# JiaruiFeng/KP-GNN

Measured on AMD Instinct MI355X. Metric: graphs/sec KP-GIN fwd+bwd, ZINC-12k K=8 L=8 h=104, higher is better.
Workload: dtype f32; 1 GPU; ZINC-12k-shaped synthetic molecules, KPGINPlus K=8 L=8 h=104 kernel=spd geometric combine, fwd+bwd+Adam, L1 loss; global_batch=2048, nodes_per_batch=47450, khop_edges_per_batch=1018372, active_pairs_per_batch=1018372, parallelism=dp1, launch=hipGraph replay of fwd+bwd, batches=4 pre-staged batches cycled

## Files before the change

include/kpgnn.h:

```cpp
#ifndef KPGNN_H_
#define KPGNN_H_

#include <stddef.h>
#include <stdint.h>

#ifdef __cplusplus
extern "C" {
#endif

#define KPGNN_ABI_VERSION 1

#define KPGNN_OK 0
#define KPGNN_EINVAL (-1)
#define KPGNN_EHIP (-2)
#define KPGNN_ELIMIT (-3)

typedef void* kpgnn_stream_t;

int kpgnn_abi_version(void);
const char* kpgnn_last_error(void);

int kpgnn_device_info(int* cu_count, int* lds_bytes_per_block, int* wavefront, char* arch, int arch_len);


// ... 341 lines not shown

#define KPGNN_STAT_REPLICAS 8
size_t kpgnn_stat_slot_bytes(int32_t C);

typedef struct kpgnn_wgrad_desc {
    int64_t N;
    int32_t O, I;
    const float* dy; int64_t dy_stride;
    const float* x;  int64_t x_stride;
    float* dw;
    float* db;
    void* workspace; size_t workspace_bytes;
    const float* x_mean; const float* x_invstd; const float* x_gamma; const float* x_beta;
    int32_t x_relu;
    kpgnn_reduce_job* defer;
    const float* dy_mask;
    const int32_t* n_dyn;
    int32_t math;
} kpgnn_wgrad_desc;

size_t kpgnn_wgrad_workspace_bytes(int32_t O, int32_t I);
int kpgnn_linear_wgrad(const kpgnn_wgrad_desc* d, kpgnn_stream_t stream);
int kpgnn_linear_wgrad_pair(const kpgnn_wgrad_desc* a, const kpgnn_wgrad_desc* b, kpgnn_stream_t stream);
size_t kpgnn_wgrad_group_workspace_bytes(int32_t O, int32_t I, int32_t group);
int kpgnn_linear_wgrad_group(const kpgnn_wgrad_desc* d, const float* const* x_group, int32_t group, kpgnn_stream_t stream);

typedef struct kpgnn_linear_desc {
    int64_t N;
    int32_t O, I;
    const float* x; int64_t x_stride;
    const float* w;
    const float* bias;
    float* y; int64_t y_stride;
    int32_t w_transposed;
    int32_t y_block_cols; int64_t y_block_stride;
    const float* x_mask;
    const int32_t* n_dyn;
    int32_t math;
    void* workspace; size_t workspace_bytes;
} kpgnn_linear_desc;

int kpgnn_linear_fwd(const kpgnn_linear_desc* d, kpgnn_stream_t stream);
size_t kpgnn_linear_split_workspace_bytes(int32_t O, int32_t I, int32_t group);
typedef struct kpgnn_split_job { const float* w; int64_t wn, wk; int32_t O, I; void* frag; } kpgnn_split_job;
int kpgnn_linear_split_many(const kpgnn_split_job* jobs, int32_t n, kpgnn_stream_t stream);

// ... 531 lines not shown
```

kp_gnn_amd/_lib.py:

```python
import ctypes
import os

import torch

_PKG = os.path.dirname(os.path.abspath(__file__))
HIP_LIB_PATH = os.path.join(_PKG, "libkpgnn_hip.so")

MODE_GIN, MODE_GINPLUS, MODE_GCN, MODE_SUM = 0, 1, 2, 3
ROUTE_SUBGROUP, ROUTE_NARROW, ROUTE_SMALL, ROUTE_LDS = 0, 1, 2, 3

c_i32, c_i64, c_f32p, c_vp = ctypes.c_int32, ctypes.c_int64, ctypes.c_void_p, ctypes.c_void_p


MATH_AUTO, MATH_F32 = 0, 1
ELIMIT = -3
DENSE_MATH = MATH_AUTO


class KpgnnError(RuntimeError):
    pass


class AggFwdDesc(ctypes.Structure):
    _fields_ = [
# ... 509 lines not shown
    "kpgnn_dict_grad_multi": (ctypes.c_int, [ctypes.POINTER(DictGradMultiDesc), c_vp]),
    "kpgnn_dict_grad_slabs": (c_i32, [c_i32]),
    "kpgnn_tile_pack_filter": (ctypes.c_int, [c_vp, c_vp, c_i64, c_i32, c_vp, c_vp, c_vp, c_vp]),
    "kpgnn_tile_pack_prefixes": (ctypes.c_int, [c_vp, c_vp, c_i64, c_i32, c_i64, c_vp, c_vp, c_vp, c_vp, c_i32, c_vp]),
    "kpgnn_collate": (ctypes.c_int, [ctypes.POINTER(CollateDesc), c_vp]),
    "kpgnn_regression_loss": (ctypes.c_int, [c_vp, c_vp, c_i64, c_i32, c_vp, c_vp, c_vp]),
    "kpgnn_score_head_fwd": (ctypes.c_int, [c_vp, c_vp, c_vp, c_i64, c_i32, c_vp, c_vp]),
    "kpgnn_score_head_bwd": (ctypes.c_int, [c_vp, c_vp, c_vp, c_i64, c_i32, c_vp, c_vp, c_vp, c_vp]),
    "kpgnn_adam_step": (ctypes.c_int, [c_vp, c_vp, c_vp, c_vp, c_i64, c_i64, ctypes.c_double, ctypes.c_double, ctypes.c_double,
                                       ctypes.c_double, ctypes.c_double, c_vp]),
    "kpgnn_reduce_jobs": (ctypes.c_int, [c_vp, c_i32, c_vp]),
    "kpgnn_adam_step_device": (ctypes.c_int, [c_vp, c_vp, c_vp, c_vp, c_i64, c_vp, ctypes.c_double, ctypes.c_double,
                                              ctypes.c_double, ctypes.c_double, ctypes.c_double, c_vp]),
    "kpgnn_multi_copy": (ctypes.c_int, [c_i32, c_vp, c_vp, c_vp, c_vp]),
    "kpgnn_dict_tile_pack": (ctypes.c_int, [c_vp, c_i64, c_i32, c_i32, c_i32, c_vp, c_vp]),
    "kpgnn_dict_tile_pack_dyn": (ctypes.c_int, [c_vp, c_i64, c_i32, c_vp, c_i32, c_i32, c_vp, c_vp]),
    "kpgnn_combine_bwd_workspace_bytes": (ctypes.c_size_t, [c_i32] * 3),
    "kpgnn_combine_bwd": (ctypes.c_int, [ctypes.POINTER(CombineBwdDesc), c_vp]),
    "kpgnn_bn_fwd": (ctypes.c_int, [ctypes.POINTER(BnDesc), c_vp]),
    "kpgnn_bn_bwd": (ctypes.c_int, [ctypes.POINTER(BnBwdDesc), c_vp]),
    "kpgnn_wgrad_workspace_bytes": (ctypes.c_size_t, [c_i32, c_i32]),
    "kpgnn_linear_wgrad": (ctypes.c_int, [ctypes.POINTER(WgradDesc), c_vp]),
    "kpgnn_linear_wgrad_pair": (ctypes.c_int, [ctypes.POINTER(WgradDesc), ctypes.POINTER(WgradDesc), c_vp]),
    "kpgnn_wgrad_group_workspace_bytes": (ctypes.c_size_t, [c_i32, c_i32, c_i32]),
    "kpgnn_linear_wgrad_group": (ctypes.c_int, [ctypes.POINTER(WgradDesc), c_vp, c_i32, c_vp]),
    "kpgnn_linear_bn": (ctypes.c_int, [ctypes.POINTER(LinearBnDesc), c_vp]),
    "kpgnn_mlp_eval": (ctypes.c_int, [ctypes.POINTER(MlpEvalDesc), c_vp]),
    "kpgnn_bn_eval": (ctypes.c_int, [ctypes.POINTER(BnEvalDesc), c_vp]),
    "kpgnn_enc_tables_fwd": (ctypes.c_int, [ctypes.POINTER(EncTablesDesc), c_vp]),
    "kpgnn_enc_tables_bwd": (ctypes.c_int, [ctypes.POINTER(EncTablesDesc), c_vp]),
    "kpgnn_segment_pool_fwd": (ctypes.c_int, [ctypes.POINTER(PoolDesc), c_vp]),
    "kpgnn_segment_pool_bwd": (ctypes.c_int, [ctypes.POINTER(PoolDesc), c_vp]),
    "kpgnn_segment_max_fwd": (ctypes.c_int, [ctypes.POINTER(PoolMaxDesc), c_vp]),
    "kpgnn_segment_max_bwd": (ctypes.c_int, [ctypes.POINTER(PoolMaxDesc), c_vp]),
    "kpgnn_resistance_distance": (ctypes.c_int, [ctypes.POINTER(RdDesc), c_vp]),
    "kpgnn_rd_large_workspace_bytes": (ctypes.c_size_t, [c_i32, c_i32]),
    "kpgnn_resistance_distance_large": (ctypes.c_int, [ctypes.POINTER(RdLargeDesc), c_vp]),
    "kpgnn_rd_proj_workspace_bytes": (ctypes.c_size_t, [c_i64, c_i32]),
    "kpgnn_rd_proj_fwd": (ctypes.c_int, [ctypes.POINTER(RdProjDesc), c_vp]),
    "kpgnn_rd_proj_bwd": (ctypes.c_int, [ctypes.POINTER(RdProjDesc), c_vp]),
    "kpgnn_khop_dev_workspace_bytes": (ctypes.c_size_t, [c_i64]),
    "kpgnn_khop_dev_count": (ctypes.c_int, [ctypes.POINTER(KhopDevDesc), c_vp]),
    "kpgnn_khop_dev_fill": (ctypes.c_int, [ctypes.POINTER(KhopDevDesc), c_vp]),
    "kpgnn_khop_large_workspace_bytes": (ctypes.c_size_t, [c_i64, c_i64, c_i32]),
    "kpgnn_khop_large_count": (ctypes.c_int, [ctypes.POINTER(KhopDevDesc), c_vp]),
    "kpgnn_khop_large_fill": (ctypes.c_int, [ctypes.POINTER(KhopDevDesc), c_vp]),
# ... 135 lines not shown
```

kp_gnn_amd/csrc/wgrad.hip:

```cpp
#include <cstdlib>
#include <type_traits>

#include "bf3.h"
#include "kpgnn_common.h"

namespace kpgnn {
namespace {

constexpr int kWgradBlocks = 512;

struct WgParams {
    int64_t N; int O, I;
    const float* dy; int64_t dys;
    const float* x; int64_t xs;
    const float* xm; const float* xi; const float* xg; const float* xb; int xrelu;
    float* slab;
    int64_t slab_row, slab_off;
};
struct WgPair { WgParams q[2]; };

template <int TI, int RG>
__device__ __forceinline__ void wgrad_problem(const WgParams p, float* lds) {
    const int lane = threadIdx.x & 63;
    const int nstrip = (int)(blockDim.x >> 6) / RG;
// ... 164 lines not shown
    switch (ti) {
        case 1: KP_WG(1); break;
        case 2: KP_WG(2); break;
        case 3: KP_WG(3); break;
        case 4: KP_WG(4); break;
        case 5: KP_WG(5); break;
        case 6: KP_WG(6); break;
        case 7: KP_WG(7); break;
        default: KP_WG(8); break;
    }
#undef KP_WG
    KPGNN_LAUNCH_CHECK("wgrad_kernel");
    return KPGNN_OK;
}

constexpr int kW2Rows = 32;
constexpr int kW2MaxProb = 16;

struct Wg2Prob {
    const float* dy; const float* x; const float* mask;
    const float* xm; const float* xi; const float* xg; const float* xb;
    int xrelu;
    int64_t dys, xs, out_off, bias_off;
};
struct Wg2Args {
    int64_t N; const int32_t* n_dyn;
    int O, I, nprob; int64_t ldw;
    float* slab; int64_t slab_row;
    Wg2Prob q[kW2MaxProb];
};

template <int TI>
__global__ void __launch_bounds__(256, 2)
wgrad2_kernel(const Wg2Args A) {
    extern __shared__ __attribute__((aligned(16))) float w2[];
    constexpr int R = kW2Rows;
    const int O = A.O, I = A.I;
    float* dyl = w2;
    float* xl = w2 + R * O;
    float* coef = xl + R * I;
    const int tid = threadIdx.x, wave = tid >> 6, lane = tid & 63;
    const int kk = lane >> 5, c = lane & 31;
    const int nprob = A.nprob;
    const int pi = (int)(blockIdx.x % nprob), slice = (int)(blockIdx.x / nprob), nslices = (int)(gridDim.x / nprob);
    Wg2Prob q = A.q[0];
#pragma unroll
    for (int i = 1; i < kW2MaxProb; ++i)
        if (pi == i) q = A.q[i];
    const int64_t N = A.n_dyn ? (int64_t)min((int64_t)*A.n_dyn, A.N) : A.N;
    const bool tr = q.xm != nullptr;
    if (tr)
// ... 57 lines not shown
#pragma unroll
    for (int t = 0; t < TI; ++t) bp[t] = xl + kk * I + min(t * 32 + c, I - 1);
    const int64_t chunks = (N + R - 1) / R;
    int64_t ch = slice;
    if (tr) __syncthreads();
    if (ch < chunks) { issue(ch); commit(ch); }
    __syncthreads();
    for (; ch < chunks; ch += nslices) {
        const int64_t nx = ch + nslices;
        const bool more = nx < chunks;
        if (more) issue(nx);
#pragma unroll
        for (int p2 = 0; p2 < R / 2; ++p2) {
            const float a = ap[2 * p2 * O];
            bsum += a;
#pragma unroll
            for (int t = 0; t < TI; ++t) acc[t] = __builtin_amdgcn_mfma_f32_32x32x2f32(a, bp[t][2 * p2 * I], acc[t], 0, 0, 0);
        }
        __syncthreads();
        if (more) commit(nx);
        __syncthreads();
    }
    bsum += __shfl_xor(bsum, 32);
    float* out = A.slab + (int64_t)slice * A.slab_row;
#pragma unroll
    for (int t = 0; t < TI; ++t) {
        const int i = t * 32 + c;
        for (int v = 0; v < 16; ++v) {
            const int orow = wave * 32 + (v & 3) + 8 * (v >> 2) + 4 * kk;
            if (orow < O && i < I) out[q.out_off + (int64_t)orow * A.ldw + i] = acc[t][v];
        }
    }
    if (q.bias_off >= 0 && kk == 0 && o_ok) out[q.bias_off + o] = bsum;
}

constexpr int kW3Pitch = 40;

constexpr int kW3Blocks = 256;

template <int TI, bool MASK>
__global__ void __launch_bounds__(512, 1)
wgrad3_kernel(const Wg2Args A) {
    extern __shared__ __attribute__((aligned(16))) float w2[];
    constexpr int R = kW2Rows, P = kW3Pitch;
    const int O = A.O, I = A.I;
    const int bufsz = 3 * (O + I) * P;
    __bf16* pl = reinterpret_cast<__bf16*>(w2);
    float* coef = reinterpret_cast<float*>(pl + 2 * bufsz);
    const int tid = threadIdx.x, lane = tid & 63;
    const int wave = __builtin_amdgcn_readfirstlane(tid >> 6);
    const int kg = lane >> 5, c = lane & 31;
    const int nprob = A.nprob;
    const int pi = (int)(blockIdx.x % nprob), slice = (int)(blockIdx.x / nprob), nslices = (int)(gridDim.x / nprob);
    Wg2Prob q = A.q[0];
#pragma unroll
    for (int i = 1; i < kW2MaxProb; ++i)
        if (pi == i) q = A.q[i];
    const int64_t N = A.n_dyn ? (int64_t)min((int64_t)*A.n_dyn, A.N) : A.N;
    const bool tr = q.xm != nullptr;
    if (tr)
        for (int i = tid; i < I; i += 512) { coef[i] = q.xm[i]; coef[I + i] = q.xi[i]; coef[2 * I + i] = q.xg[i]; coef[3 * I + i] = q.xb[i]; }
    const int64_t chunks = (N + R - 1) / R;
    const int64_t mine = slice < chunks ? (chunks - slice + nslices - 1) / nslices : 0;
    const bool producer = wave >= 4;
    const bool is_x = wave >= 6;
    const int ncg = (is_x ? I : O) >> 2;
    const int task = tid & 127;
    const bool owner = producer && task < 4 * ncg;
    const int g = owner ? task & 3 : 0, cg = owner ? task >> 2 : 0;
    const float* src = is_x ? q.x : q.dy;
    const int64_t sstride = is_x ? q.xs : q.dys;
    const uint32_t sbytes = (uint32_t)sstride * 4u;
    const bool xform = tr && is_x;
    const int64_t last = N - 1;
    bf3_f2 bs01 = {0.f, 0.f}, bs23 = {0.f, 0.f};
    auto produce = [&](auto mask_c) {
        constexpr bool M = decltype(mask_c)::value;
        float4 pv0[8], pm0[8], pv1[8], pm1[8];
        auto issue = [&](int64_t k, float4 (&pv)[8], float4 (&pm)[8]) {
            const int64_t c0 = (slice + min(k, mine - 1) * nslices) * R;
            const float* cp = src + c0 * sstride;
            const float* mp = M ? q.mask + c0 * sstride : nullptr;
            const int lim = (int)min((int64_t)R, N - c0) - 1;
#pragma unroll
            for (int j = 0; j < 8; ++j) {
                const uint32_t off = __umul24((uint32_t)min(8 * g + j, lim), sbytes) + 16u * (uint32_t)cg;
                pv[j] = *reinterpret_cast<const float4*>(reinterpret_cast<const char*>(cp) + off);
                if (M) pm[j] = *reinterpret_cast<const float4*>(reinterpret_cast<const char*>(mp) + off);
            }
        };
        auto commit = [&](int64_t k, float4 (&pv)[8], float4 (&pm)[8]) {
            const int64_t c0 = (slice + min(k, mine - 1) * nslices) * R;
            if (M) {
    #pragma unroll
                for (int j = 0; j < 8; ++j) {
                    pv[j].x = pm[j].x > 0.f ? pv[j].x : 0.f; pv[j].y = pm[j].y > 0.f ? pv[j].y : 0.f;
                    pv[j].z = pm[j].z > 0.f ? pv[j].z : 0.f; pv[j].w = pm[j].w > 0.f ? pv[j].w : 0.f;
                }
            }
            if (xform) {
                const float4 m4 = *reinterpret_cast<const float4*>(coef + 4 * cg), s4 = *reinterpret_cast<const float4*>(coef + I + 4 * cg);
                const float4 g4 = *reinterpret_cast<const float4*>(coef + 2 * I + 4 * cg), b4 = *reinterpret_cast<const float4*>(coef + 3 * I + 4 * cg);
    #pragma unroll
                for (int j = 0; j < 8; ++j) {
                    float4 v = pv[j];
                    v.x = fmaf((v.x - m4.x) * s4.x, g4.x, b4.x); v.y = fmaf((v.y - m4.y) * s4.y, g4.y, b4.y);
                    v.z = fmaf((v.z - m4.z) * s4.z, g4.z, b4.z); v.w = fmaf((v.w - m4.w) * s4.w, g4.w, b4.w);
                    if (q.xrelu) { v.x = fmaxf(v.x, 0.f); v.y = fmaxf(v.y, 0.f); v.z = fmaxf(v.z, 0.f); v.w = fmaxf(v.w, 0.f); }
                    pv[j] = v;
                }
            }
            if (c0 + R > N) {
    #pragma unroll
                for (int j = 0; j < 8; ++j)
                    if (c0 + 8 * g + j >= N) pv[j] = make_float4(0.f, 0.f, 0.f, 0.f);
            }
            if (!is_x && k < mine) {
    #pragma unroll
                for (int j = 0; j < 8; ++j) { bs01 += bf3_f2{pv[j].x, pv[j].y}; bs23 += bf3_f2{pv[j].z, pv[j].w}; }
            }
            if (owner) {
                __bf16* base = pl + (k & 1) * bufsz + (is_x ? 3 * O * P : 0) + 8 * g;
                const int cols = is_x ? I : O;
    #pragma unroll
                for (int e2 = 0; e2 < 2; ++e2) {
                    bf3_u2 h[8], m[8], l[8];
#pragma unroll
                    for (int j = 0; j < 8; ++j)
                        bf3_split2(e2 == 0 ? bf3_f2{pv[j].x, pv[j].y} : bf3_f2{pv[j].z, pv[j].w}, h[j], m[j], l[j]);
                    __bf16* col = base + (4 * cg + 2 * e2) * P;
                    *reinterpret_cast<uint4*>(col) = make_uint4(bf3_pack(h[0].x, h[1].x), bf3_pack(h[2].x, h[3].x), bf3_pack(h[4].x, h[5].x), bf3_pack(h[6].x, h[7].x));
                    *reinterpret_cast<uint4*>(col + P) = make_uint4(bf3_pack(h[0].y, h[1].y), bf3_pack(h[2].y, h[3].y), bf3_pack(h[4].y, h[5].y), bf3_pack(h[6].y, h[7].y));
                    *reinterpret_cast<uint4*>(col + cols * P) = make_uint4(bf3_pack(m[0].x, m[1].x), bf3_pack(m[2].x, m[3].x), bf3_pack(m[4].x, m[5].x), bf3_pack(m[6].x, m[7].x));
                    *reinterpret_cast<uint4*>(col + cols * P + P) = make_uint4(bf3_pack(m[0].y, m[1].y), bf3_pack(m[2].y, m[3].y), bf3_pack(m[4].y, m[5].y), bf3_pack(m[6].y, m[7].y));
                    *reinterpret_cast<uint4*>(col + 2 * cols * P) = make_uint4(bf3_pack(l[0].x, l[1].x), bf3_pack(l[2].x, l[3].x), bf3_pack(l[4].x, l[5].x), bf3_pack(l[6].x, l[7].x));
                    *reinterpret_cast<uint4*>(col + 2 * cols * P + P) = make_uint4(bf3_pack(l[0].y, l[1].y), bf3_pack(l[2].y, l[3].y), bf3_pack(l[4].y, l[5].y), bf3_pack(l[6].y, l[7].y));
                }
            }
        };
        __builtin_amdgcn_s_setprio(2);
        if (mine > 0) {
            issue(0, pv0, pm0);
            issue(1, pv1, pm1);
            commit(0, pv0, pm0);
            issue(2, pv0, pm0);
        }
        __syncthreads();
        for (int64_t k = 0; k < mine; k += 2) {
            commit(k + 1, pv1, pm1);
            issue(k + 3, pv1, pm1);
            __syncthreads();
            commit(k + 2, pv0, pm0);
            issue(k + 4, pv0, pm0);
            __syncthreads();
        }
    };
    f32x16 acc[TI];
#pragma unroll
    for (int t = 0; t < TI; ++t)
        for (int v = 0; v < 16; ++v) acc[t][v] = 0.f;
    const int o = wave * 32 + c;
    const bool strip = !producer && wave * 32 < O;
    const int aoff = min(o, O - 1) * P + 8 * kg;
    int boff[TI];
#pragma unroll
    for (int t = 0; t < TI; ++t) boff[t] = 3 * O * P + min(t * 32 + c, I - 1) * P + 8 * kg;
    auto ld8 = [&](const __bf16* ptr) { return __builtin_bit_cast(bf3_x8, *reinterpret_cast<const uint4*>(ptr)); };
    auto multiply = [&](int64_t k) {
        const __bf16* bf = pl + (k & 1) * bufsz;
#pragma unroll
        for (int ks = 0; ks < R / 16; ++ks) {
            const bf3_x8 ah = ld8(bf + aoff + 16 * ks), am = ld8(bf + aoff + O * P + 16 * ks), al = ld8(bf + aoff + 2 * O * P + 16 * ks);
            bf3_x8 bh[TI], bm[TI], bl[TI];
#pragma unroll
            for (int t = 0; t < TI; ++t) {
                bh[t] = ld8(bf + boff[t] + 16 * ks); bm[t] = ld8(bf + boff[t] + I * P + 16 * ks); bl[t] = ld8(bf + boff[t] + 2 * I * P + 16 * ks);
            }
#pragma unroll
            for (int t = 0; t < TI; ++t) acc[t] = __builtin_amdgcn_mfma_f32_32x32x16_bf16(al, bh[t], acc[t], 0, 0, 0);
#pragma unroll
            for (int t = 0; t < TI; ++t) acc[t] = __builtin_amdgcn_mfma_f32_32x32x16_bf16(ah, bl[t], acc[t], 0, 0, 0);
#pragma unroll
            for (int t = 0; t < TI; ++t) acc[t] = __builtin_amdgcn_mfma_f32_32x32x16_bf16(am, bm[t], acc[t], 0, 0, 0);
#pragma unroll
            for (int t = 0; t < TI; ++t) acc[t] = __builtin_amdgcn_mfma_f32_32x32x16_bf16(am, bh[t], acc[t], 0, 0, 0);
#pragma unroll
            for (int t = 0; t < TI; ++t) acc[t] = __builtin_amdgcn_mfma_f32_32x32x16_bf16(ah, bm[t], acc[t], 0, 0, 0);
#pragma unroll
            for (int t = 0; t < TI; ++t) acc[t] = __builtin_amdgcn_mfma_f32_32x32x16_bf16(ah, bh[t], acc[t], 0, 0, 0);
        }
    };
    if (tr) __syncthreads();
    float* out = A.slab + (int64_t)slice * A.slab_row;
    if (producer) {
        if (MASK && !is_x) produce(std::true_type{});
        else produce(std::false_type{});
    } else {
        __syncthreads();
        for (int64_t k = 0; k < mine; k += 2) {
            if (strip) multiply(k);

            __syncthreads();

            if (strip && k + 1 < mine) multiply(k + 1);

            __syncthreads();
        }
        if (strip) {
#pragma unroll
            for (int t = 0; t < TI; ++t) {
                const int i = t * 32 + c;
                for (int v = 0; v < 16; ++v) {
                    const int orow = wave * 32 + (v & 3) + 8 * (v >> 2) + 4 * kg;
                    if (orow < O && i < I) out[q.out_off + (int64_t)orow * A.ldw + i] = acc[t][v];
                }
            }
        }
    }
    if (q.bias_off >= 0) {
        if (owner && !is_x) *reinterpret_cast<float4*>(coef + g * O + 4 * cg) = make_float4(bs01.x, bs01.y, bs23.x, bs23.y);
        __syncthreads();
        if (tid < O) out[q.bias_off + tid] = (coef[tid] + coef[O + tid]) + (coef[2 * O + tid] + coef[3 * O + tid]);
    }
}

bool wgrad3_ok(const Wg2Args& A) {
    for (int i = 1; i < A.nprob; ++i)
        if ((A.q[i].mask != nullptr) != (A.q[0].mask != nullptr)) return false;
    for (int i = 0; i < A.nprob; ++i)
        if (A.q[i].dys >= (1 << 22) || A.q[i].xs >= (1 << 22)) return false;
    return A.O <= 128 && A.I <= 128;
}
size_t wgrad3_lds(const Wg2Args& A) {
    const int m = A.O > A.I ? A.O : A.I;
    return (size_t)2 * 2 * 3 * (A.O + A.I) * kW3Pitch + sizeof(float) * 4 * (size_t)m;
}

bool wgrad2_ok(const kpgnn_wgrad_desc* d, const float* x) {
    auto al = [](const void* q) { return (((uintptr_t)q) & 15) == 0; };
    return d->O % 4 == 0 && d->I % 4 == 0 && d->O <= 128 && d->I <= 256 && d->dy_stride % 4 == 0 && d->x_stride % 4 == 0 &&
           al(d->dy) && al(x) && (!d->dy_mask || al(d->dy_mask));
}

Wg2Prob wgrad2_prob(const kpgnn_wgrad_desc* d, const float* x, int64_t out_off, int64_t bias_off) {
    Wg2Prob q;
    q.dy = d->dy; q.x = x; q.mask = d->dy_mask; q.xm = d->x_mean; q.xi = d->x_invstd; q.xg = d->x_gamma; q.xb = d->x_beta;
    q.xrelu = d->x_relu; q.dys = d->dy_stride; q.xs = d->x_stride; q.out_off = out_off; q.bias_off = bias_off;
    return q;
}

int wgrad2_slices(int64_t N, int nprob, int blocks) {
    const int64_t chunks = (N + kW2Rows - 1) / kW2Rows;
    int64_t s = blocks / nprob;
    if (s > chunks) s = chunks;
    return (int)(s < 1 ? 1 : s);
}

int wgrad2_launch(Wg2Args& A, int math, int* nslices, hipStream_t s) {
    const int ti = (A.I + 31) / 32;
    if (math != KPGNN_MATH_F32 && wgrad3_ok(A)) {
        *nslices = wgrad2_slices(A.N, A.nprob, kW3Blocks);
        dim3 gr3((unsigned)(*nslices * A.nprob)), blk3(512);
        const size_t lds3 = wgrad3_lds(A);
        const bool mask = A.q[0].mask != nullptr;
#define KP_W3(T) do { if (mask) { KPGNN_HIP_TRY(ensure_dynamic_lds((const void*)wgrad3_kernel<T, true>, lds3)); \
                                  hipLaunchKernelGGL((wgrad3_kernel<T, true>), gr3, blk3, lds3, s, A); } \
                      else { KPGNN_HIP_TRY(ensure_dynamic_lds((const void*)wgrad3_kernel<T, false>, lds3)); \
                             hipLaunchKernelGGL((wgrad3_kernel<T, false>), gr3, blk3, lds3, s, A); } } while (0)
        switch (ti) {
            case 1: KP_W3(1); break;
            case 2: KP_W3(2); break;
            case 3: KP_W3(3); break;
            default: KP_W3(4); break;
        }
#undef KP_W3
        KPGNN_LAUNCH_CHECK("wgrad3_kernel");
        return KPGNN_OK;
    }
    *nslices = wgrad2_slices(A.N, A.nprob, kWgradBlocks);
    dim3 gr((unsigned)(*nslices * A.nprob)), blk(256);
    const size_t lds = sizeof(float) * ((size_t)kW2Rows * (A.O + A.I) + 4 * (size_t)A.I);
#define KP_W2(T) hipLaunchKernelGGL((wgrad2_kernel<T>), gr, blk, lds, s, A)
    switch (ti) {
        case 1: KP_W2(1); break;
        case 2: KP_W2(2); break;
        case 3: KP_W2(3); break;
        case 4: KP_W2(4); break;
        case 5: KP_W2(5); break;
        case 6: KP_W2(6); break;
        case 7: KP_W2(7); break;
        default: KP_W2(8); break;
    }
#undef KP_W2
    KPGNN_LAUNCH_CHECK("wgrad2_kernel");
    return KPGNN_OK;
}

}
}

using namespace kpgnn;

extern "C" size_t kpgnn_wgrad_workspace_bytes(int32_t O, int32_t I) {
    if (O < 1 || I < 1) return 0;
    return sizeof(float) * ((size_t)kWgradBlocks * ((size_t)O * I + O) + O);
}

extern "C" int kpgnn_linear_wgrad(const kpgnn_wgrad_desc* d, kpgnn_stream_t stream) {
    int rc = wgrad_check(d, "linear_wgrad");
    if (rc != KPGNN_OK) return rc;
    KPGNN_REQUIRE(d->workspace && d->workspace_bytes >= kpgnn_wgrad_workspace_bytes(d->O, d->I), "linear_wgrad: workspace too small");
    const int64_t nw = (int64_t)d->O * d->I;
    float* slab = (float*)d->workspace;
    hipStream_t s = (hipStream_t)stream;
    int grid;
    if (wgrad2_ok(d, d->x)) {
        Wg2Args A;
        A.N = d->N; A.n_dyn = d->n_dyn; A.O = d->O; A.I = d->I; A.nprob = 1; A.ldw = d->I; A.slab = slab; A.slab_row = nw + d->O;
        for (int i = 0; i < kW2MaxProb; ++i) A.q[i] = wgrad2_prob(d, d->x, 0, nw);
        rc = wgrad2_launch(A, d->math, &grid, s);
    } else {
        KPGNN_REQUIRE(!d->dy_mask && !d->n_dyn, "linear_wgrad: dy_mask / n_dyn need 16-B aligned operands with O %% 4 == I %% 4 == 0, O <= 128");
        WgPair pp;
        pp.q[0] = pp.q[1] = wgrad_params(d, slab, nw + d->O, 0);
        grid = wgrad_blocks(d->N, d->O);
        rc = wgrad_launch(pp, 1, d->O, d->I, grid, s);
    }
    if (rc != KPGNN_OK) return rc;
    float* db = d->db ? d->db : slab + (size_t)kWgradBlocks * (nw + d->O);
    if (d->defer) {
        kpgnn_reduce_job* j = d->defer;
        j->slab = slab; j->nslab = grid; j->elems = nw + d->O;
        j->out[0] = d->dw; j->n_out[0] = nw; j->out[1] = db; j->n_out[1] = d->O;
        j->out[2] = j->out[3] = nullptr; j->n_out[2] = j->n_out[3] = 0;
        return KPGNN_OK;
    }
    return slab_reduce(slab, grid, nw + d->O, d->dw, nw, db, d->O, nullptr, s);
}

extern "C" int kpgnn_linear_wgrad_pair(const kpgnn_wgrad_desc* a, const kpgnn_wgrad_desc* b, kpgnn_stream_t stream) {
    int rc = wgrad_check(a, "linear_wgrad_pair");
    if (rc != KPGNN_OK) return rc;
    rc = wgrad_check(b, "linear_wgrad_pair");
    if (rc != KPGNN_OK) return rc;
    KPGNN_REQUIRE(a->O == b->O && a->I == b->I && a->N == b->N, "linear_wgrad_pair: the two problems must share N, O, I");
    KPGNN_REQUIRE(a->db && b->db, "linear_wgrad_pair: both bias gradients are required");
    KPGNN_REQUIRE(a->workspace && a->workspace_bytes >= 2 * kpgnn_wgrad_workspace_bytes(a->O, a->I), "linear_wgrad_pair: workspace too small");
    const int64_t nw = (int64_t)a->O * a->I, one = nw + a->O;
    float* slab = (float*)a->workspace;
    hipStream_t s = (hipStream_t)stream;
    int grid;
    if (wgrad2_ok(a, a->x) && wgrad2_ok(b, b->x)) {
        Wg2Args A;
        A.N = a->N; A.n_dyn = a->n_dyn; A.O = a->O; A.I = a->I; A.nprob = 2; A.ldw = a->I; A.slab = slab; A.slab_row = 2 * one;
        for (int i = 0; i < kW2MaxProb; ++i) A.q[i] = wgrad2_prob(a, a->x, 0, nw);
        A.q[1] = wgrad2_prob(b, b->x, one, one + nw);
        rc = wgrad2_launch(A, a->math, &grid, s);
    } else {
        KPGNN_REQUIRE(!a->dy_mask && !b->dy_mask && !a->n_dyn, "linear_wgrad_pair: dy_mask / n_dyn need 16-B aligned operands");
        WgPair pp;
        pp.q[0] = wgrad_params(a, slab, 2 * one, 0);
        pp.q[1] = wgrad_params(b, slab, 2 * one, one);
        grid = wgrad_blocks(a->N, a->O);
        rc = wgrad_launch(pp, 2, a->O, a->I, grid, s);
    }
    if (rc != KPGNN_OK) return rc;
    if (a->defer) {
        kpgnn_reduce_job* j = a->defer;
        j->slab = slab; j->nslab = grid; j->elems = 2 * one;
        j->out[0] = a->dw; j->n_out[0] = nw; j->out[1] = a->db; j->n_out[1] = a->O;
        j->out[2] = b->dw; j->n_out[2] = nw; j->out[3] = b->db; j->n_out[3] = b->O;
        return KPGNN_OK;
    }
    return slab_reduce(slab, grid, 2 * one, a->dw, nw, a->db, a->O, b->dw, s, nw, b->db);
}

extern "C" size_t kpgnn_wgrad_group_workspace_bytes(int32_t O, int32_t I, int32_t group) {
    if (O < 1 || I < 1 || group < 1 || group > kW2MaxProb) return 0;
    return sizeof(float) * ((size_t)(kWgradBlocks / group) * ((size_t)O * I * group + O) + O);
}

extern "C" int kpgnn_linear_wgrad_group(const kpgnn_wgrad_desc* d, const float* const* x_group, int32_t group, kpgnn_stream_t stream) {
    KPGNN_REQUIRE(d != nullptr && x_group != nullptr && group >= 1 && group <= kW2MaxProb, "linear_wgrad_group: bad arguments (1 <= group <= %d)", kW2MaxProb);
    kpgnn_wgrad_desc probe = *d;
    probe.x = x_group[0];
    int rc = wgrad_check(&probe, "linear_wgrad_group");
    if (rc != KPGNN_OK) return rc;
    for (int l = 0; l < group; ++l)
        if (!x_group[l] || !wgrad2_ok(d, x_group[l]))
            return fail(KPGNN_ELIMIT, "linear_wgrad_group: needs 16-B aligned operands, O %% 4 == I %% 4 == 0, O <= 128, I <= 256");
    KPGNN_REQUIRE(!d->x_mean, "linear_wgrad_group: no x transform");
    KPGNN_REQUIRE(d->workspace && d->workspace_bytes >= kpgnn_wgrad_group_workspace_bytes(d->O, d->I, group), "linear_wgrad_group: workspace too small");
    const int64_t nw = (int64_t)d->O * d->I * group;
    Wg2Args A;
    A.N = d->N; A.n_dyn = d->n_dyn; A.O = d->O; A.I = d->I; A.nprob = group; A.ldw = (int64_t)d->I * group;
    A.slab = (float*)d->workspace; A.slab_row = nw + d->O;
    for (int i = 0; i < kW2MaxProb; ++i) A.q[i] = wgrad2_prob(d, x_group[i < group ? i : 0], (int64_t)(i < group ? i : 0) * d->I, i == 0 ? nw : -1);
    int grid = 0;
    hipStream_t s = (hipStream_t)stream;
    rc = wgrad2_launch(A, d->math, &grid, s);
    if (rc != KPGNN_OK) return rc;
    float* db = d->db ? d->db : A.slab + (size_t)grid * A.slab_row;
    if (d->defer) {
        kpgnn_reduce_job* j = d->defer;
        j->slab = A.slab; j->nslab = grid; j->elems = nw + d->O;
        j->out[0] = d->dw; j->n_out[0] = nw; j->out[1] = db; j->n_out[1] = d->O;
        j->out[2] = j->out[3] = nullptr; j->n_out[2] = j->n_out[3] = 0;
        return KPGNN_OK;
    }
    return slab_reduce(A.slab, grid, nw + d->O, d->dw, nw, db, d->O, nullptr, s);
}
```

kp_gnn_amd/ops.py:

```python
import collections
import ctypes

import numpy as np
import torch

from . import _lib
from ._lib import MODE_GCN, MODE_GIN, MODE_GINPLUS, MODE_SUM, LaunchTimer, set_launch_timer
from .ops_dataset import (COUNT_LABELS_AUTO, GRAPH_LABELS_AUTO, count_labels, count_labels_launch, graph_labels_launch,
                          graph_property_labels, khop_transform, resistance_distance)

_SQRT1_2 = 0.7071067811865476
_INV_SQRT_2PI = 0.3989422804014327


def algorithmic_bytes(csr, k_act, D, n_tensors, n_rows_tables, extra_nd=0, s=4):
    A = csr.active_pairs(k_act)
    return int(s * csr.N * k_act * D * n_tensors) + A * 6 + 4 * (csr.N * csr.K + 1) + 4 * D * n_rows_tables \
        + 4 * csr.N * D * extra_nd


_STORAGE = torch.float32


def set_storage_dtype(dtype):
# ... 52 lines not shown


def _last_contig(t):
    return t if t.stride(-1) == 1 else t.contiguous()


def _require_cuda(*ts):
    for t in ts:
        if t is not None and not t.is_cuda:
            raise _lib.KpgnnError("kp_gnn_amd ops need CUDA/HIP tensors: there is no CPU fallback "
                                  "(the CPU restatement lives in oracle/ and is test-only)")


def _check_codes(csr, k_act, table0, tablek):
    if csr.A == 0:
        return
    if csr.max_code0 >= table0.shape[0]:
        raise IndexError(f"edge code {csr.max_code0} out of range for hop1_edge_emb with {table0.shape[0]} rows")
    if k_act > 1 and tablek is not None and csr.max_codek >= tablek.shape[0]:
        raise IndexError(f"edge code {csr.max_codek} out of range for hopk_edge_emb with {tablek.shape[0]} rows")


_pending_reduce = None


class deferred_reductions:
    def __enter__(self):
        global _pending_reduce
        self._outer = _pending_reduce
        if _pending_reduce is None:
            _pending_reduce = []
        return self

    def __exit__(self, *exc):
        global _pending_reduce
        if self._outer is None:
            jobs, _pending_reduce = _pending_reduce, None
            _deferred_owners.clear()
            if jobs and exc[0] is None:
                flush_reductions(jobs)
        return False


def flush_reductions(jobs):
    arr = (_lib.ReduceJob * len(jobs))(*[j for j, _ in jobs])
    _lib.launch("kpgnn_reduce_jobs", jobs[0][1][0].device, arr, len(jobs))


_deferred_owners = set()


def defer_reduce_job(*params):
    if _pending_reduce is None:
        return None
    keys = {p.data_ptr() for p in params if p is not None}
    if keys & _deferred_owners:
        jobs = list(_pending_reduce)
        del _pending_reduce[:]
        _deferred_owners.clear()
        if jobs:
            flush_reductions(jobs)
        return None
    _deferred_owners.update(keys)
    return _lib.ReduceJob()


def queue_reduce_job(job, keep_alive):
    _pending_reduce.append((job, keep_alive))


def take_reduce_job():
    if _pending_reduce:
        return _pending_reduce.pop(0)
    return None


class DictPeripheral:

    def __init__(self, table, uid):
        self.table, self.uid = table, uid

    @property
    def shape(self):
        return (self.uid.shape[0], self.uid.shape[1], self.table.shape[1])

    def __getitem__(self, idx):
        if (isinstance(idx, tuple) and len(idx) == 2 and idx[0] == slice(None) and isinstance(idx[1], slice)
# ... 2032 lines not shown
```

kp_gnn_amd/ops_dense.py:

```python
import ctypes

import torch
import torch.nn.functional as F

from . import _lib
from .ops import _ptr, dyn_ptr, refuse_dynamic_rows


STAT_REPLICAS = 8
_EAGER_DOUBLES = 1 << 20
_GRAPH_DOUBLES = 1 << 18


class _Arena:
    __slots__ = ("buf", "off", "end")

    def __init__(self, n, dev):
        self.buf = torch.zeros(n, dtype=torch.float64, device=dev)
        self.off, self.end = 0, n // 2


_arenas = {}


# ... 411 lines not shown
        okw = dict(pro=3, o_mean=st[4], o_invstd=st[5], o_gamma=gO, o_dgamma=gb[4], o_dbeta=gb[5]) if ctx.outer else dict(pro=2)
        _lin_bn(lib, dev, N=N, O=O, I=O, x=dz, w=w3, y=da1, w_transposed=1, epi=2, pro_relu=1, in_slot=slot2,
                in_gamma=g2, in_beta=be2, in_mean=st[2], in_invstd=st[3], x2=y2, xt=dy2, dgamma=gb[0], dbeta=gb[1],
                out_slot=slot1, e_x=y1, e_mean=st[0], e_invstd=st[1], e_gamma=g1, e_beta=be1, **okw)
        _lin_bn(lib, dev, N=N, O=I, I=O, x=da1, w=w0, y=dh, w_transposed=1, pro=2, epi=0, pro_relu=0, in_slot=slot1,
                in_gamma=g1, in_beta=be1, in_mean=st[0], in_invstd=st[1], x2=y1, xt=dy1, dgamma=gb[2], dbeta=gb[3])
        dw3 = torch.empty((O, O), dtype=torch.float32, device=dev)
        dw0 = torch.empty((O, I), dtype=torch.float32, device=dev)
        db = torch.empty((2, O), dtype=torch.float32, device=dev)
        a, b = _lib.WgradDesc(), _lib.WgradDesc()
        a.N, a.O, a.I = N, O, O
        a.n_dyn = b.n_dyn = dyn_ptr(N)
        a.dy, a.dy_stride, a.x, a.x_stride = dy2.data_ptr(), O, y1.data_ptr(), O
        a.dw, a.db = dw3.data_ptr(), db[0].data_ptr()
        a.x_mean, a.x_invstd, a.x_gamma, a.x_beta, a.x_relu = st[0].data_ptr(), st[1].data_ptr(), g1.data_ptr(), be1.data_ptr(), 1
        b.N, b.O, b.I = N, O, I
        b.dy, b.dy_stride, b.x, b.x_stride = dy1.data_ptr(), O, h.data_ptr(), I
        b.dw, b.db = dw0.data_ptr(), db[1].data_ptr()
        if I == O:
            from . import ops
            nb = 2 * int(lib.kpgnn_wgrad_workspace_bytes(O, O))
            ws = torch.empty(nb, dtype=torch.uint8, device=dev)
            a.workspace, a.workspace_bytes = ws.data_ptr(), nb
            job = ops.defer_reduce_job(w0, w3)
            if job is not None:
                a.defer = ctypes.cast(ctypes.pointer(job), ctypes.c_void_p)
            _lib.launch("kpgnn_linear_wgrad_pair", dev, ctypes.byref(a), ctypes.byref(b))
            if job is not None:
                ops.queue_reduce_job(job, (ws, dw3, dw0, db))
        else:
            for q in (a, b):
                nb = int(lib.kpgnn_wgrad_workspace_bytes(q.O, q.I))
                ws = torch.empty(nb, dtype=torch.uint8, device=dev)
                q.workspace, q.workspace_bytes = ws.data_ptr(), nb
                _lib.launch("kpgnn_linear_wgrad", dev, ctypes.byref(q))
        gres = dz if (ctx.outer and ctx.has_res and rbuf is None and not handed) else None
        return (dh if ctx.needs_input_grad[0] else None, dw0, db[1] if ctx.has_b0 else None, gb[2], gb[3],
                dw3, db[0] if ctx.has_b3 else None, gb[0], gb[1], None, None, None,
                gb[4] if ctx.outer else None, gb[5] if ctx.outer else None, gres, None)


def _fusable_bn(bn):
    return bn.training and bn.affine and bn.momentum is not None


def mlp_linear_bn_relu_x2(mlp, h, emit_out_stats=False, post_norm=None):
    l0, bn1, l3, bn2 = mlp[0], mlp[1], mlp[3], mlp[4]
    O, I = l0.weight.shape
    bnO, res = post_norm if post_norm is not None else (None, None)
    if (not torch.is_grad_enabled() and h.is_cuda and h.dim() == 2 and h.dtype == torch.float32 and h.shape[0] >= 1
            and _eval_bn(bn1) and _eval_bn(bn2) and (bnO is None or _eval_bn(bnO)) and tuple(l3.weight.shape) == (O, O)
            and _eval_residual_ok(res, (h.shape[0], O))):
# ... 516 lines not shown
```

Measured before the change: 681,300 graphs/s.

## Batch MLP weight-gradient pairs across layers into one multi-problem wgrad3 launch

MLP weight-gradient pairs are now parked during backward instead of launched one layer at a time. Up to 8 layers are then flushed in a single kernel launch that handles up to 16 problems, each writing to its own slab. The wgrad3 kernel gains a cursor scheme so a block can cover several slices of one problem, dumping accumulators and bias partials at each slice boundary. This is meant to cut launch count and raise occupancy for small 104x104 wgrads, at the cost of delaying gradient computation, holding activations alive longer, and more complex per-block bookkeeping.

```diff
diff --git a/include/kpgnn.h b/include/kpgnn.h
--- a/include/kpgnn.h
+++ b/include/kpgnn.h
@@ -387,6 +387,8 @@
 size_t kpgnn_wgrad_workspace_bytes(int32_t O, int32_t I);
 int kpgnn_linear_wgrad(const kpgnn_wgrad_desc* d, kpgnn_stream_t stream);
 int kpgnn_linear_wgrad_pair(const kpgnn_wgrad_desc* a, const kpgnn_wgrad_desc* b, kpgnn_stream_t stream);
+int kpgnn_linear_wgrad_many(const kpgnn_wgrad_desc* const* a, const kpgnn_wgrad_desc* const* b, int32_t count,
+                            kpgnn_stream_t stream);
 size_t kpgnn_wgrad_group_workspace_bytes(int32_t O, int32_t I, int32_t group);
 int kpgnn_linear_wgrad_group(const kpgnn_wgrad_desc* d, const float* const* x_group, int32_t group, kpgnn_stream_t stream);
 
diff --git a/kp_gnn_amd/_lib.py b/kp_gnn_amd/_lib.py
--- a/kp_gnn_amd/_lib.py
+++ b/kp_gnn_amd/_lib.py
@@ -555,6 +555,8 @@
     "kpgnn_wgrad_workspace_bytes": (ctypes.c_size_t, [c_i32, c_i32]),
     "kpgnn_linear_wgrad": (ctypes.c_int, [ctypes.POINTER(WgradDesc), c_vp]),
     "kpgnn_linear_wgrad_pair": (ctypes.c_int, [ctypes.POINTER(WgradDesc), ctypes.POINTER(WgradDesc), c_vp]),
+    "kpgnn_linear_wgrad_many": (ctypes.c_int, [ctypes.POINTER(ctypes.POINTER(WgradDesc)), ctypes.POINTER(ctypes.POINTER(WgradDesc)),
+                                               c_i32, c_vp]),
     "kpgnn_wgrad_group_workspace_bytes": (ctypes.c_size_t, [c_i32, c_i32, c_i32]),
     "kpgnn_linear_wgrad_group": (ctypes.c_int, [ctypes.POINTER(WgradDesc), c_vp, c_i32, c_vp]),
     "kpgnn_linear_bn": (ctypes.c_int, [ctypes.POINTER(LinearBnDesc), c_vp]),
diff --git a/kp_gnn_amd/csrc/wgrad.hip b/kp_gnn_amd/csrc/wgrad.hip
--- a/kp_gnn_amd/csrc/wgrad.hip
+++ b/kp_gnn_amd/csrc/wgrad.hip
@@ -210,11 +210,13 @@
     const float* xm; const float* xi; const float* xg; const float* xb;
     int xrelu;
     int64_t dys, xs, out_off, bias_off;
+    float* slab;
 };
 struct Wg2Args {
     int64_t N; const int32_t* n_dyn;
     int O, I, nprob; int64_t ldw;
-    float* slab; int64_t slab_row;
+    int64_t slab_row;
+    int nslices;
     Wg2Prob q[kW2MaxProb];
 };
 
@@ -318,7 +320,7 @@
         __syncthreads();
     }
     bsum += __shfl_xor(bsum, 32);
-    float* out = A.slab + (int64_t)slice * A.slab_row;
+    float* out = q.slab + (int64_t)slice * A.slab_row;
 #pragma unroll
     for (int t = 0; t < TI; ++t) {
         const int i = t * 32 + c;
@@ -347,7 +349,7 @@
     const int wave = __builtin_amdgcn_readfirstlane(tid >> 6);
     const int kg = lane >> 5, c = lane & 31;
     const int nprob = A.nprob;
-    const int pi = (int)(blockIdx.x % nprob), slice = (int)(blockIdx.x / nprob), nslices = (int)(gridDim.x / nprob);
+    const int pi = (int)(blockIdx.x % nprob), pb = (int)(blockIdx.x / nprob), G = (int)(gridDim.x / nprob), nslices = A.nslices;
     Wg2Prob q = A.q[0];
 #pragma unroll
     for (int i = 1; i < kW2MaxProb; ++i)
@@ -357,7 +359,24 @@
     if (tr)
         for (int i = tid; i < I; i += 512) { coef[i] = q.xm[i]; coef[I + i] = q.xi[i]; coef[2 * I + i] = q.xg[i]; coef[3 * I + i] = q.xb[i]; }
     const int64_t chunks = (N + R - 1) / R;
-    const int64_t mine = slice < chunks ? (chunks - slice + nslices - 1) / nslices : 0;
+    const int nch = (int)chunks;
+    const int slim = min(nslices, nch);
+    const int nv = (nslices - pb + G - 1) / G;
+    const int nfull = pb < slim ? (slim - pb + G - 1) / G : 0;
+    int total = 0;
+    {
+        const int m = (nch + nslices - 1) / nslices, rem = nch - (m - 1) * nslices;
+        const int nm = pb < rem ? (rem - pb + G - 1) / G : 0;
+        total = nch > 0 ? nv * (m - 1) + nm : 0;
+    }
+    struct Cur { int s, c; };
+    auto ends = [&](const Cur& cu) { return cu.c + nslices >= nch; };
+    auto step = [&](Cur& cu) {
+        const bool wrap = ends(cu), go = wrap && cu.s + G < slim;
+        cu.s = go ? cu.s + G : cu.s;
+        cu.c = wrap ? (go ? cu.s : cu.c) : cu.c + nslices;
+    };
+    const Cur first = {pb, pb};
     const bool producer = wave >= 4;
     const bool is_x = wave >= 6;
     const int ncg = (is_x ? I : O) >> 2;
@@ -370,11 +389,27 @@
     const bool xform = tr && is_x;
     const int64_t last = N - 1;
     bf3_f2 bs01 = {0.f, 0.f}, bs23 = {0.f, 0.f};
+    auto bias_out = [&](int s) {
+        float b4[4] = {bs01.x, bs01.y, bs23.x, bs23.y};
+#pragma unroll
+        for (int e = 0; e < 4; ++e) {
+            b4[e] += __shfl_xor(b4[e], 1);
+            b4[e] += __shfl_xor(b4[e], 2);
+        }
+        if (q.bias_off >= 0 && owner && g == 0) {
+            float* bo = q.slab + (int64_t)s * A.slab_row + q.bias_off + 4 * cg;
+#pragma unroll
+            for (int e = 0; e < 4; ++e) bo[e] = b4[e];
+        }
+        bs01 = bf3_f2{0.f, 0.f}; bs23 = bf3_f2{0.f, 0.f};
+    };
     auto produce = [&](auto mask_c) {
         constexpr bool M = decltype(mask_c)::value;
         float4 pv0[8], pm0[8], pv1[8], pm1[8];
-        auto issue = [&](int64_t k, float4 (&pv)[8], float4 (&pm)[8]) {
-            const int64_t c0 = (slice + min(k, mine - 1) * nslices) * R;
+        Cur ic = first, cc = first;
+        auto issue = [&](float4 (&pv)[8], float4 (&pm)[8]) {
+            const int64_t c0 = (int64_t)ic.c * R;
+            step(ic);
             const float* cp = src + c0 * sstride;
             const float* mp = M ? q.mask + c0 * sstride : nullptr;
             const int lim = (int)min((int64_t)R, N - c0) - 1;
@@ -385,8 +420,8 @@
                 if (M) pm[j] = *reinterpret_cast<const float4*>(reinterpret_cast<const char*>(mp) + off);
             }
         };
-        auto commit = [&](int64_t k, float4 (&pv)[8], float4 (&pm)[8]) {
-            const int64_t c0 = (slice + min(k, mine - 1) * nslices) * R;
+        auto commit = [&](int k, float4 (&pv)[8], float4 (&pm)[8]) {
+            const int64_t c0 = (int64_t)cc.c * R;
             if (M) {
     #pragma unroll
                 for (int j = 0; j < 8; ++j) {
@@ -411,9 +446,10 @@
                 for (int j = 0; j < 8; ++j)
                     if (c0 + 8 * g + j >= N) pv[j] = make_float4(0.f, 0.f, 0.f, 0.f);
             }
-            if (!is_x && k < mine) {
+            if (!is_x && k < total) {
     #pragma unroll
                 for (int j = 0; j < 8; ++j) { bs01 += bf3_f2{pv[j].x, pv[j].y}; bs23 += bf3_f2{pv[j].z, pv[j].w}; }
+                if (ends(cc)) bias_out(cc.s);
             }
             if (owner) {
                 __bf16* base = pl + (k & 1) * bufsz + (is_x ? 3 * O * P : 0) + 8 * g;
@@ -433,23 +469,26 @@
                     *reinterpret_cast<uint4*>(col + 2 * cols * P + P) = make_uint4(bf3_pack(l[0].y, l[1].y), bf3_pack(l[2].y, l[3].y), bf3_pack(l[4].y, l[5].y), bf3_pack(l[6].y, l[7].y));
                 }
             }
+            step(cc);
         };
         __builtin_amdgcn_s_setprio(2);
-        if (mine > 0) {
-            issue(0, pv0, pm0);
-            issue(1, pv1, pm1);
+        if (total > 0) {
+            issue(pv0, pm0);
+            issue(pv1, pm1);
             commit(0, pv0, pm0);
-            issue(2, pv0, pm0);
+            issue(pv0, pm0);
         }
         __syncthreads();
-        for (int64_t k = 0; k < mine; k += 2) {
+        for (int k = 0; k < total; k += 2) {
             commit(k + 1, pv1, pm1);
-            issue(k + 3, pv1, pm1);
+            issue(pv1, pm1);
             __syncthreads();
             commit(k + 2, pv0, pm0);
-            issue(k + 4, pv0, pm0);
+            issue(pv0, pm0);
             __syncthreads();
         }
+        if (!is_x)
+            for (int v = nfull; v < nv; ++v) bias_out(pb + v * G);
     };
     f32x16 acc[TI];
 #pragma unroll
@@ -462,7 +501,7 @@
 #pragma unroll
     for (int t = 0; t < TI; ++t) boff[t] = 3 * O * P + min(t * 32 + c, I - 1) * P + 8 * kg;
     auto ld8 = [&](const __bf16* ptr) { return __builtin_bit_cast(bf3_x8, *reinterpret_cast<const uint4*>(ptr)); };
-    auto multiply = [&](int64_t k) {
+    auto multiply = [&](int k) {
         const __bf16* bf = pl + (k & 1) * bufsz;
 #pragma unroll
         for (int ks = 0; ks < R / 16; ++ks) {
@@ -487,36 +526,44 @@
         }
     };
     if (tr) __syncthreads();
-    float* out = A.slab + (int64_t)slice * A.slab_row;
+    auto dump = [&](int s) {
+        if (!strip) return;
+        float* out = q.slab + (int64_t)s * A.slab_row + q.out_off;
+        int Od = O, Id = I;
+        asm volatile("" : "+s"(Od), "+s"(Id));
+#pragma unroll
+        for (int t = 0; t < TI; ++t) {
+            const int i = t * 32 + c;
+#pragma unroll
+            for (int v = 0; v < 16; ++v) {
+                const int orow = wave * 32 + (v & 3) + 8 * (v >> 2) + 4 * kg;
+                if (orow < Od && i < Id) out[(int64_t)orow * A.ldw + i] = acc[t][v];
+                acc[t][v] = 0.f;
+            }
+        }
+    };
     if (producer) {
         if (MASK && !is_x) produce(std::true_type{});
         else produce(std::false_type{});
     } else {
+        Cur mc = first;
         __syncthreads();
-        for (int64_t k = 0; k < mine; k += 2) {
+        for (int k = 0; k < total; k += 2) {
             if (strip) multiply(k);
-
+            const bool end0 = ends(mc);
+            const int s0 = mc.s;
+            step(mc);
             __syncthreads();
-
-            if (strip && k + 1 < mine) multiply(k + 1);
-
+            if (end0) dump(s0);
+            const bool more = k + 1 < total;
+            if (strip && more) multiply(k + 1);
+            const bool end1 = more && ends(mc);
+            const int s1 = mc.s;
+            step(mc);
             __syncthreads();
-        }
-        if (strip) {
-#pragma unroll
-            for (int t = 0; t < TI; ++t) {
-                const int i = t * 32 + c;
-                for (int v = 0; v < 16; ++v) {
-                    const int orow = wave * 32 + (v & 3) + 8 * (v >> 2) + 4 * kg;
-                    if (orow < O && i < I) out[q.out_off + (int64_t)orow * A.ldw + i] = acc[t][v];
-                }
-            }
-        }
-    }
-    if (q.bias_off >= 0) {
-        if (owner && !is_x) *reinterpret_cast<float4*>(coef + g * O + 4 * cg) = make_float4(bs01.x, bs01.y, bs23.x, bs23.y);
-        __syncthreads();
-        if (tid < O) out[q.bias_off + tid] = (coef[tid] + coef[O + tid]) + (coef[2 * O + tid] + coef[3 * O + tid]);
+            if (end1) dump(s1);
+        }
+        for (int v = nfull; v < nv; ++v) dump(pb + v * G);
     }
 }
 
@@ -538,8 +585,9 @@
            al(d->dy) && al(x) && (!d->dy_mask || al(d->dy_mask));
 }
 
-Wg2Prob wgrad2_prob(const kpgnn_wgrad_desc* d, const float* x, int64_t out_off, int64_t bias_off) {
+Wg2Prob wgrad2_prob(const kpgnn_wgrad_desc* d, const float* x, int64_t out_off, int64_t bias_off, float* slab) {
     Wg2Prob q;
+    q.slab = slab;
     q.dy = d->dy; q.x = x; q.mask = d->dy_mask; q.xm = d->x_mean; q.xi = d->x_invstd; q.xg = d->x_gamma; q.xb = d->x_beta;
     q.xrelu = d->x_relu; q.dys = d->dy_stride; q.xs = d->x_stride; q.out_off = out_off; q.bias_off = bias_off;
     return q;
@@ -552,11 +600,10 @@
     return (int)(s < 1 ? 1 : s);
 }
 
-int wgrad2_launch(Wg2Args& A, int math, int* nslices, hipStream_t s) {
+int wgrad3_launch(const Wg2Args& A, int per_prob, hipStream_t s) {
     const int ti = (A.I + 31) / 32;
-    if (math != KPGNN_MATH_F32 && wgrad3_ok(A)) {
-        *nslices = wgrad2_slices(A.N, A.nprob, kW3Blocks);
-        dim3 gr3((unsigned)(*nslices * A.nprob)), blk3(512);
+    {
+        dim3 gr3((unsigned)(per_prob * A.nprob)), blk3(512);
         const size_t lds3 = wgrad3_lds(A);
         const bool mask = A.q[0].mask != nullptr;
 #define KP_W3(T) do { if (mask) { KPGNN_HIP_TRY(ensure_dynamic_lds((const void*)wgrad3_kernel<T, true>, lds3)); \
@@ -573,7 +620,15 @@
         KPGNN_LAUNCH_CHECK("wgrad3_kernel");
         return KPGNN_OK;
     }
-    *nslices = wgrad2_slices(A.N, A.nprob, kWgradBlocks);
+}
+
+int wgrad2_launch(Wg2Args& A, int math, int* nslices, hipStream_t s) {
+    const int ti = (A.I + 31) / 32;
+    if (math != KPGNN_MATH_F32 && wgrad3_ok(A)) {
+        *nslices = A.nslices = wgrad2_slices(A.N, A.nprob, kW3Blocks);
+        return wgrad3_launch(A, *nslices, s);
+    }
+    *nslices = A.nslices = wgrad2_slices(A.N, A.nprob, kWgradBlocks);
     dim3 gr((unsigned)(*nslices * A.nprob)), blk(256);
     const size_t lds = sizeof(float) * ((size_t)kW2Rows * (A.O + A.I) + 4 * (size_t)A.I);
 #define KP_W2(T) hipLaunchKernelGGL((wgrad2_kernel<T>), gr, blk, lds, s, A)
@@ -612,8 +667,8 @@
     int grid;
     if (wgrad2_ok(d, d->x)) {
         Wg2Args A;
-        A.N = d->N; A.n_dyn = d->n_dyn; A.O = d->O; A.I = d->I; A.nprob = 1; A.ldw = d->I; A.slab = slab; A.slab_row = nw + d->O;
-        for (int i = 0; i < kW2MaxProb; ++i) A.q[i] = wgrad2_prob(d, d->x, 0, nw);
+        A.N = d->N; A.n_dyn = d->n_dyn; A.O = d->O; A.I = d->I; A.nprob = 1; A.ldw = d->I; A.slab_row = nw + d->O;
+        for (int i = 0; i < kW2MaxProb; ++i) A.q[i] = wgrad2_prob(d, d->x, 0, nw, slab);
         rc = wgrad2_launch(A, d->math, &grid, s);
     } else {
         KPGNN_REQUIRE(!d->dy_mask && !d->n_dyn, "linear_wgrad: dy_mask / n_dyn need 16-B aligned operands with O %% 4 == I %% 4 == 0, O <= 128");
@@ -648,9 +703,9 @@
     int grid;
     if (wgrad2_ok(a, a->x) && wgrad2_ok(b, b->x)) {
         Wg2Args A;
-        A.N = a->N; A.n_dyn = a->n_dyn; A.O = a->O; A.I = a->I; A.nprob = 2; A.ldw = a->I; A.slab = slab; A.slab_row = 2 * one;
-        for (int i = 0; i < kW2MaxProb; ++i) A.q[i] = wgrad2_prob(a, a->x, 0, nw);
-        A.q[1] = wgrad2_prob(b, b->x, one, one + nw);
+        A.N = a->N; A.n_dyn = a->n_dyn; A.O = a->O; A.I = a->I; A.nprob = 2; A.ldw = a->I; A.slab_row = 2 * one;
+        for (int i = 0; i < kW2MaxProb; ++i) A.q[i] = wgrad2_prob(a, a->x, 0, nw, slab);
+        A.q[1] = wgrad2_prob(b, b->x, one, one + nw, slab);
         rc = wgrad2_launch(A, a->math, &grid, s);
     } else {
         KPGNN_REQUIRE(!a->dy_mask && !b->dy_mask && !a->n_dyn, "linear_wgrad_pair: dy_mask / n_dyn need 16-B aligned operands");
@@ -669,6 +724,59 @@
         return KPGNN_OK;
     }
     return slab_reduce(slab, grid, 2 * one, a->dw, nw, a->db, a->O, b->dw, s, nw, b->db);
+}
+
+extern "C" int kpgnn_linear_wgrad_many(const kpgnn_wgrad_desc* const* a, const kpgnn_wgrad_desc* const* b, int32_t count,
+                                       kpgnn_stream_t stream) {
+    KPGNN_REQUIRE(a != nullptr && b != nullptr && count >= 1 && 2 * count <= kW2MaxProb,
+                  "linear_wgrad_many: bad arguments (1 <= count <= %d)", kW2MaxProb / 2);
+    for (int p = 0; p < count; ++p) KPGNN_REQUIRE(a[p] && b[p], "linear_wgrad_many: pair %d is missing", p);
+    bool one = count > 1 && a[0]->math != KPGNN_MATH_F32;
+    for (int p = 0; p < count && one; ++p) {
+        const kpgnn_wgrad_desc *x = a[p], *y = b[p];
+        one = wgrad_check(x, "linear_wgrad_many") == KPGNN_OK && wgrad_check(y, "linear_wgrad_many") == KPGNN_OK &&
+              x->N == a[0]->N && y->N == a[0]->N && x->O == a[0]->O && y->O == a[0]->O && x->I == a[0]->I && y->I == a[0]->I &&
+              x->n_dyn == a[0]->n_dyn && y->n_dyn == a[0]->n_dyn && x->math == a[0]->math && x->db && y->db &&
+              x->workspace && x->workspace_bytes >= 2 * kpgnn_wgrad_workspace_bytes(x->O, x->I) &&
+              wgrad2_ok(x, x->x) && wgrad2_ok(y, y->x);
+    }
+    Wg2Args A;
+    int64_t nw = 0, row = 0;
+    if (one) {
+        nw = (int64_t)a[0]->O * a[0]->I; row = nw + a[0]->O;
+        A.N = a[0]->N; A.n_dyn = a[0]->n_dyn; A.O = a[0]->O; A.I = a[0]->I; A.nprob = 2 * count; A.ldw = a[0]->I; A.slab_row = 2 * row;
+        for (int i = 0; i < kW2MaxProb; ++i) {
+            const int p = i < 2 * count ? i / 2 : 0;
+            float* slab = (float*)a[p]->workspace;
+            A.q[i] = i % 2 == 0 ? wgrad2_prob(a[p], a[p]->x, 0, nw, slab) : wgrad2_prob(b[p], b[p]->x, row, row + nw, slab);
+        }
+        one = wgrad3_ok(A);
+    }
+    if (!one) {
+        for (int p = 0; p < count; ++p) {
+            const int rc = kpgnn_linear_wgrad_pair(a[p], b[p], stream);
+            if (rc != KPGNN_OK) return rc;
+        }
+        return KPGNN_OK;
+    }
+    hipStream_t s = (hipStream_t)stream;
+    A.nslices = wgrad2_slices(A.N, 2, kW3Blocks);
+    const int per_prob = A.nslices < kW3Blocks / A.nprob ? A.nslices : kW3Blocks / A.nprob;
+    int rc = wgrad3_launch(A, per_prob, s);
+    if (rc != KPGNN_OK) return rc;
+    for (int p = 0; p < count; ++p) {
+        float* slab = (float*)a[p]->workspace;
+        if (a[p]->defer) {
+            kpgnn_reduce_job* j = a[p]->defer;
+            j->slab = slab; j->nslab = A.nslices; j->elems = 2 * row;
+            j->out[0] = a[p]->dw; j->n_out[0] = nw; j->out[1] = a[p]->db; j->n_out[1] = A.O;
+            j->out[2] = b[p]->dw; j->n_out[2] = nw; j->out[3] = b[p]->db; j->n_out[3] = A.O;
+            continue;
+        }
+        rc = slab_reduce(slab, A.nslices, 2 * row, a[p]->dw, nw, a[p]->db, A.O, b[p]->dw, s, nw, b[p]->db);
+        if (rc != KPGNN_OK) return rc;
+    }
+    return KPGNN_OK;
 }
 
 extern "C" size_t kpgnn_wgrad_group_workspace_bytes(int32_t O, int32_t I, int32_t group) {
@@ -690,19 +798,20 @@
     const int64_t nw = (int64_t)d->O * d->I * group;
     Wg2Args A;
     A.N = d->N; A.n_dyn = d->n_dyn; A.O = d->O; A.I = d->I; A.nprob = group; A.ldw = (int64_t)d->I * group;
-    A.slab = (float*)d->workspace; A.slab_row = nw + d->O;
-    for (int i = 0; i < kW2MaxProb; ++i) A.q[i] = wgrad2_prob(d, x_group[i < group ? i : 0], (int64_t)(i < group ? i : 0) * d->I, i == 0 ? nw : -1);
+    float* slab = (float*)d->workspace;
+    A.slab_row = nw + d->O;
+    for (int i = 0; i < kW2MaxProb; ++i) A.q[i] = wgrad2_prob(d, x_group[i < group ? i : 0], (int64_t)(i < group ? i : 0) * d->I, i == 0 ? nw : -1, slab);
     int grid = 0;
     hipStream_t s = (hipStream_t)stream;
     rc = wgrad2_launch(A, d->math, &grid, s);
     if (rc != KPGNN_OK) return rc;
-    float* db = d->db ? d->db : A.slab + (size_t)grid * A.slab_row;
+    float* db = d->db ? d->db : slab + (size_t)grid * A.slab_row;
     if (d->defer) {
         kpgnn_reduce_job* j = d->defer;
-        j->slab = A.slab; j->nslab = grid; j->elems = nw + d->O;
+        j->slab = slab; j->nslab = grid; j->elems = nw + d->O;
         j->out[0] = d->dw; j->n_out[0] = nw; j->out[1] = db; j->n_out[1] = d->O;
         j->out[2] = j->out[3] = nullptr; j->n_out[2] = j->n_out[3] = 0;
         return KPGNN_OK;
     }
-    return slab_reduce(A.slab, grid, nw + d->O, d->dw, nw, db, d->O, nullptr, s);
-}
+    return slab_reduce(slab, grid, nw + d->O, d->dw, nw, db, d->O, nullptr, s);
+}
diff --git a/kp_gnn_amd/ops.py b/kp_gnn_amd/ops.py
--- a/kp_gnn_amd/ops.py
+++ b/kp_gnn_amd/ops.py
@@ -98,6 +98,8 @@
 
 
 _pending_reduce = None
+_parked_wgrad = []
+WGRAD_MANY_PAIRS = 8
 
 
 class deferred_reductions:
@@ -111,6 +113,9 @@
     def __exit__(self, *exc):
         global _pending_reduce
         if self._outer is None:
+            if exc[0] is None:
+                flush_parked_wgrad()
+            del _parked_wgrad[:]
             jobs, _pending_reduce = _pending_reduce, None
             _deferred_owners.clear()
             if jobs and exc[0] is None:
@@ -131,6 +136,7 @@
         return None
     keys = {p.data_ptr() for p in params if p is not None}
     if keys & _deferred_owners:
+        flush_parked_wgrad()
         jobs = list(_pending_reduce)
         del _pending_reduce[:]
         _deferred_owners.clear()
@@ -139,6 +145,43 @@
         return None
     _deferred_owners.update(keys)
     return _lib.ReduceJob()
+
+
+def park_wgrad_pair(a, b, params, keep_alive):
+    if _pending_reduce is None or a.math == _lib.MATH_F32 or a.O != a.I or a.O > 128 or a.O % 4:
+        return False
+    keys = {p.data_ptr() for p in params}
+    if keys & _deferred_owners:
+        return False
+    shape = (a.N, a.O, a.I, a.n_dyn, keep_alive[0].device)
+    if _parked_wgrad and _parked_wgrad[0][0] != shape:
+        flush_parked_wgrad()
+    _deferred_owners.update(keys)
+    _parked_wgrad.append((shape, a, b, keys, keep_alive))
+    if len(_parked_wgrad) == WGRAD_MANY_PAIRS:
+        flush_parked_wgrad()
+    return True
+
+
+def flush_parked_wgrad():
+    parked = list(_parked_wgrad)
+    del _parked_wgrad[:]
+    if not parked:
+        return
+    dev = parked[0][0][-1]
+    jobs = []
+    for _, a, _, keys, keep_alive in parked:
+        job = _lib.ReduceJob()
+        a.defer = ctypes.cast(ctypes.pointer(job), ctypes.c_void_p)
+        jobs.append((job, keep_alive))
+        _deferred_owners.difference_update(keys)
+    if len(parked) == 1:
+        _lib.launch("kpgnn_linear_wgrad_pair", dev, ctypes.byref(parked[0][1]), ctypes.byref(parked[0][2]))
+    else:
+        ptrs = ctypes.POINTER(_lib.WgradDesc) * len(parked)
+        _lib.launch("kpgnn_linear_wgrad_many", dev, ptrs(*[ctypes.pointer(e[1]) for e in parked]),
+                    ptrs(*[ctypes.pointer(e[2]) for e in parked]), len(parked))
+    flush_reductions(jobs)
 
 
 def queue_reduce_job(job, keep_alive):
diff --git a/kp_gnn_amd/ops_dense.py b/kp_gnn_amd/ops_dense.py
--- a/kp_gnn_amd/ops_dense.py
+++ b/kp_gnn_amd/ops_dense.py
@@ -457,12 +457,13 @@
             nb = 2 * int(lib.kpgnn_wgrad_workspace_bytes(O, O))
             ws = torch.empty(nb, dtype=torch.uint8, device=dev)
             a.workspace, a.workspace_bytes = ws.data_ptr(), nb
-            job = ops.defer_reduce_job(w0, w3)
-            if job is not None:
-                a.defer = ctypes.cast(ctypes.pointer(job), ctypes.c_void_p)
-            _lib.launch("kpgnn_linear_wgrad_pair", dev, ctypes.byref(a), ctypes.byref(b))
-            if job is not None:
-                ops.queue_reduce_job(job, (ws, dw3, dw0, db))
+            if not ops.park_wgrad_pair(a, b, (w0, w3), (ws, dw3, dw0, db, dy2, dy1, y1, h, st, g1, be1)):
+                job = ops.defer_reduce_job(w0, w3)
+                if job is not None:
+                    a.defer = ctypes.cast(ctypes.pointer(job), ctypes.c_void_p)
+                _lib.launch("kpgnn_linear_wgrad_pair", dev, ctypes.byref(a), ctypes.byref(b))
+                if job is not None:
+                    ops.queue_reduce_job(job, (ws, dw3, dw0, db))
         else:
             for q in (a, b):
                 nb = int(lib.kpgnn_wgrad_workspace_bytes(q.O, q.I))
```

Measured after the change: 690,000 graphs/s, median of 6. 1.01x the previous value.
